# NVIDIA-Merlin/models

Hardware: NVIDIA H100
Metric: DLRM fwd samples/sec (Criteo shape, batch 65536/GPU) (higher is better)
Workload: dtype fp32 I/O; GEMM-shaped work as split-bf16 x3 (hi*hi + hi*lo + lo*hi, fp32 accumulate, |err| ~ 2^-16)

## Files before the change

### models_b200/csrc/mlp_tc.cu

```cuda
#include <cuda.h>
#include <cuda_bf16.h>

#include <cstring>

#include "mm_common.cuh"
#include "tc_common.cuh"

namespace mm {
namespace mlp {

using namespace mm::tc;

constexpr int BLOCK_M = 128;
constexpr int BLOCK_K = 64;
constexpr int MMA_K = 16;
constexpr int kConsumerWarps = 8;
constexpr int kThreads = 32 * (kConsumerWarps + 1);
constexpr int kMaxChain = 3;
constexpr int kMaxHeads = 8;
constexpr uint32_t A_TILE_BYTES = BLOCK_M * BLOCK_K * 2;

struct ChainLayer {
  int N, Np;
  int Kp;
  int act;
  uint32_t w_off;
};

struct Params {
  long long M;
  int K1p, N1, N1p, act1, stages, n_chain;
  ChainLayer c[kMaxChain];
  const float* bias[kMaxChain + 1];
  uint32_t w_bytes;
  float* out_f32;
  uint8_t* out_operand;
  long long out_stride;
  const float* head_w;
  float head_b;
  int head_act;
  float* head_out;
  int n_heads;
  const float* heads_w;
  const float* heads_b;
  int heads_act[kMaxHeads];
  float* heads_out;
};

template <int NP, int KS>
__device__ __forceinline__ void chain_mma(float (&acc)[64], const uint32_t (&ahi)[32], const uint32_t (&alo)[32], uint32_t w_hi,
                                          uint32_t w_lo, uint32_t tile_b) {
  wgmma_fence();
#pragma unroll
  for (int ks = 0; ks < KS; ++ks) {
    const uint32_t f[4] = {ahi[4 * ks], ahi[4 * ks + 1], ahi[4 * ks + 2], ahi[4 * ks + 3]};
    wgmma_rs(NP, acc, f, make_desc_sw128(w_lo + (ks >> 2) * tile_b + (ks & 3) * 32));
  }
#pragma unroll
  for (int ks = 0; ks < KS; ++ks) {
    const uint32_t f[4] = {alo[4 * ks], alo[4 * ks + 1], alo[4 * ks + 2], alo[4 * ks + 3]};
    wgmma_rs(NP, acc, f, make_desc_sw128(w_hi + (ks >> 2) * tile_b + (ks & 3) * 32));
  }
#pragma unroll
  for (int ks = 0; ks < KS; ++ks) {
    const uint32_t f[4] = {ahi[4 * ks], ahi[4 * ks + 1], ahi[4 * ks + 2], ahi[4 * ks + 3]};
    wgmma_rs(NP, acc, f, make_desc_sw128(w_hi + (ks >> 2) * tile_b + (ks & 3) * 32));
  }
  wgmma_commit();
  wgmma_wait_all();
}
template <int KS>
__device__ __forceinline__ void chain_mma(int np, float (&acc)[64], const uint32_t (&ahi)[32], const uint32_t (&alo)[32],
                                          uint32_t w_hi, uint32_t w_lo, uint32_t tile_b) {
  switch (np) {
    case 16: chain_mma<16, KS>(acc, ahi, alo, w_hi, w_lo, tile_b); break;
    case 32: chain_mma<32, KS>(acc, ahi, alo, w_hi, w_lo, tile_b); break;
    case 48: chain_mma<48, KS>(acc, ahi, alo, w_hi, w_lo, tile_b); break;
    case 64: chain_mma<64, KS>(acc, ahi, alo, w_hi, w_lo, tile_b); break;
    case 80: chain_mma<80, KS>(acc, ahi, alo, w_hi, w_lo, tile_b); break;
    case 96: chain_mma<96, KS>(acc, ahi, alo, w_hi, w_lo, tile_b); break;
    case 112: chain_mma<112, KS>(acc, ahi, alo, w_hi, w_lo, tile_b); break;
    default: chain_mma<128, KS>(acc, ahi, alo, w_hi, w_lo, tile_b); break;
  }
}

template <int N1P, bool HEADS>
__global__ void __launch_bounds__(kThreads, 1)
mlp_tc_kernel(const __grid_constant__ CUtensorMap tmA, const __grid_constant__ CUtensorMap tmW1,
              const __grid_constant__ CUtensorMap tmC0, const __grid_constant__ CUtensorMap tmC1,
              const __grid_constant__ CUtensorMap tmC2, const Params p) {
  extern __shared__ __align__(1024) uint8_t smem_raw[];
  uint8_t* smem = smem_raw + ((1024u - (smem_u32(smem_raw) & 1023u)) & 1023u);
  constexpr uint32_t B_TILE_BYTES = (uint32_t)N1P * BLOCK_K * 2;
  constexpr uint32_t STAGE_BYTES = A_TILE_BYTES + B_TILE_BYTES;
  uint8_t* wres = smem + (size_t)p.stages * STAGE_BYTES;
  uint64_t* bars = reinterpret_cast<uint64_t*>(wres + p.w_bytes);
  uint64_t* full_bar = bars;
  uint64_t* empty_bar = bars + p.stages;
  uint64_t* w_full = bars + 2 * p.stages;
  float* bias_s = reinterpret_cast<float*>(bars + 2 * p.stages + 2);
  float* head_s = bias_s + (kMaxChain + 1) * 128;

  const int warp = threadIdx.x >> 5, lane = threadIdx.x & 31;
  const long long tiles = (p.M + BLOCK_M - 1) / BLOCK_M;
  const int KB = p.K1p / BLOCK_K;

  if (warp == kConsumerWarps && lane == 0) {
    asm volatile("prefetch.tensormap [%0];" ::"l"(&tmA) : "memory");
    asm volatile("prefetch.tensormap [%0];" ::"l"(&tmW1) : "memory");
    for (int s = 0; s < p.stages; ++s) {
      mbar_init(smem_u32(full_bar + s), 1);
      mbar_init(smem_u32(empty_bar + s), kConsumerWarps);
    }
    mbar_init(smem_u32(w_full), 1);
    asm volatile("fence.mbarrier_init.release.cluster;" ::: "memory");
  }
  for (int i = threadIdx.x; i < (kMaxChain + 1) * 128; i += kThreads) {
    const int l = i >> 7, n = i & 127;
    const int N = l == 0 ? p.N1 : (l <= p.n_chain ? p.c[l - 1].N : 0);
    bias_s[i] = (p.bias[l] != nullptr && n < N) ? p.bias[l][n] : 0.0f;
  }
  if (HEADS) {
    const int Nl = p.n_chain ? p.c[p.n_chain - 1].N : p.N1;
    for (int i = threadIdx.x; i < kMaxHeads * 128; i += kThreads) {
      const int hh = i >> 7, n = i & 127;
      head_s[i] = (hh < p.n_heads && n < Nl) ? p.heads_w[n * p.n_heads + hh] : 0.0f;
    }
    if (threadIdx.x < kMaxHeads)
      head_s[kMaxHeads * 128 + threadIdx.x] = ((int)threadIdx.x < p.n_heads && p.heads_b) ? p.heads_b[threadIdx.x] : 0.0f;
  } else if (threadIdx.x < 128) {
    const int Nl = p.n_chain ? p.c[p.n_chain - 1].N : p.N1;
    head_s[threadIdx.x] = (p.head_w != nullptr && (int)threadIdx.x < Nl) ? p.head_w[threadIdx.x] : 0.0f;
  }
  __syncthreads();

  if (warp == kConsumerWarps) {
    if (lane == 0) {
      if (p.n_chain > 0) {
        const uint32_t wb = smem_u32(w_full);
        mbar_expect_tx(wb, p.w_bytes);
        for (int c = 0; c < p.n_chain; ++c) {
          const CUtensorMap* tm = c == 0 ? &tmC0 : (c == 1 ? &tmC1 : &tmC2);
          const uint32_t tile_b = (uint32_t)p.c[c].Np * BLOCK_K * 2;
          const int kbs = p.c[c].Kp / BLOCK_K;
          for (int kb = 0; kb < kbs; ++kb) {
            tma_load_2d(smem_u32(wres + p.c[c].w_off + (size_t)kb * tile_b), tm, wb, kb * BLOCK_K, 0);
            tma_load_2d(smem_u32(wres + p.c[c].w_off + (size_t)(kbs + kb) * tile_b), tm, wb, p.c[c].Kp + kb * BLOCK_K, 0);
          }
        }
      }
      int stage = 0;
      uint32_t phase = 0;
      for (long long tile = blockIdx.x; tile < tiles; tile += gridDim.x) {
        const int m0 = (int)tile * BLOCK_M;
        for (int kb2 = 0; kb2 < 2 * KB; ++kb2) {
          const int kb = kb2 >> 1, col = (kb2 & 1) * p.K1p + kb * BLOCK_K;
          mbar_wait(smem_u32(empty_bar + stage), phase ^ 1);
          const uint32_t fb = smem_u32(full_bar + stage);
          uint8_t* st = smem + (size_t)stage * STAGE_BYTES;
          mbar_expect_tx(fb, STAGE_BYTES);
          tma_load_2d(smem_u32(st), &tmA, fb, col, m0);
          tma_load_2d(smem_u32(st + A_TILE_BYTES), &tmW1, fb, col, 0);
          if (++stage == p.stages) {
            stage = 0;
            phase ^= 1;
          }
        }
      }
    }
  } else {
    const int wg = warp >> 2;
    const int c2 = 2 * (lane & 3);
    const int frow = 64 * wg + 16 * (warp & 3) + (lane >> 2);
    const uint32_t a_off = (uint32_t)wg * (A_TILE_BYTES / 2);
    int stage = 0;
    uint32_t phase = 0;
    bool weights_ready = p.n_chain == 0;
    for (long long tile = blockIdx.x; tile < tiles; tile += gridDim.x) {
      float acc[64];
#pragma unroll
      for (int i = 0; i < 64; ++i) acc[i] = 0.0f;
      for (int kb = 0; kb < KB; ++kb) {
        const int s_hi = stage;
        mbar_wait(smem_u32(full_bar + s_hi), phase);
        const uint32_t a_hi = smem_u32(smem + (size_t)s_hi * STAGE_BYTES), b_hi = a_hi + A_TILE_BYTES;
        wgmma_fence_acc(acc);
        wgmma_fence();
#pragma unroll
        for (int k = 0; k < BLOCK_K / MMA_K; ++k)
          wgmma_ss(N1P, acc, make_desc_sw128(a_hi + a_off + k * 32), make_desc_sw128(b_hi + k * 32));
        wgmma_commit();
        if (++stage == p.stages) {
          stage = 0;
          phase ^= 1;
        }
        const int s_lo = stage;
        mbar_wait(smem_u32(full_bar + s_lo), phase);
        const uint32_t a_lo = smem_u32(smem + (size_t)s_lo * STAGE_BYTES), b_lo = a_lo + A_TILE_BYTES;
        wgmma_fence();
#pragma unroll
        for (int k = 0; k < BLOCK_K / MMA_K; ++k)
          wgmma_ss(N1P, acc, make_desc_sw128(a_hi + a_off + k * 32), make_desc_sw128(b_lo + k * 32));
#pragma unroll
        for (int k = 0; k < BLOCK_K / MMA_K; ++k)
          wgmma_ss(N1P, acc, make_desc_sw128(a_lo + a_off + k * 32), make_desc_sw128(b_hi + k * 32));
        wgmma_commit();
        wgmma_wait_all();
        wgmma_fence_acc(acc);
        __syncwarp();
        if (lane == 0) {
          mbar_arrive(smem_u32(empty_bar + s_hi));
          mbar_arrive(smem_u32(empty_bar + s_lo));
        }
        if (++stage == p.stages) {
          stage = 0;
          phase ^= 1;
        }
      }

      for (int layer = 0; layer <= p.n_chain; ++layer) {
        const bool last = layer == p.n_chain;
        const int N = layer == 0 ? p.N1 : p.c[layer - 1].N;
        const int Np = layer == 0 ? N1P : p.c[layer - 1].Np;
        const int act = layer == 0 ? p.act1 : p.c[layer - 1].act;
        const float* bs = bias_s + layer * 128;
#pragma unroll
        for (int j = 0; j < 16; ++j) {
          if (8 * j < Np) {
#pragma unroll
            for (int e = 0; e < 4; ++e) {
              const int col = 8 * j + c2 + (e & 1);
              float v = acc[4 * j + e] + bs[col];
              if (act == MM_ACT_RELU) v = fmaxf(v, 0.0f);
              else if (act != MM_ACT_LINEAR && col < N) v = apply_act_slow(v, act);
              acc[4 * j + e] = col < N ? v : 0.0f;
            }
          }
        }
        if (!last) {
          uint32_t ahi[32], alo[32];
#pragma unroll
          for (int i = 0; i < 32; ++i) split_pair(acc[2 * i], acc[2 * i + 1], ahi[i], alo[i]);
          const ChainLayer& L = p.c[layer];
          if (!weights_ready) {
            mbar_wait(smem_u32(w_full), 0);
            weights_ready = true;
          }
          const uint32_t tile_b = (uint32_t)L.Np * BLOCK_K * 2;
          const uint32_t w_hi = smem_u32(wres + L.w_off), w_lo = w_hi + (uint32_t)(L.Kp / BLOCK_K) * tile_b;
#pragma unroll
          for (int i = 0; i < 64; ++i) acc[i] = 0.0f;
          wgmma_fence_acc(acc);
          if (L.Kp == BLOCK_K) chain_mma<BLOCK_K / MMA_K>(L.Np, acc, ahi, alo, w_hi, w_lo, tile_b);
          else chain_mma<2 * BLOCK_K / MMA_K>(L.Np, acc, ahi, alo, w_hi, w_lo, tile_b);
          wgmma_fence_acc(acc);
        } else {
#pragma unroll
          for (int h = 0; h < 2; ++h) {
            const long long row = tile * BLOCK_M + frow + 8 * h;
            if (HEADS) {
#pragma unroll
              for (int hh = 0; hh < kMaxHeads; ++hh) {
                if (hh < p.n_heads) {
                  const float* hw = head_s + hh * 128;
                  float hsum = 0.0f;
#pragma unroll
                  for (int j = 0; j < 4; ++j) {
                    hsum = fmaf(acc[4 * j + 2 * h], hw[8 * j + c2], hsum);
                    hsum = fmaf(acc[4 * j + 2 * h + 1], hw[8 * j + c2 + 1], hsum);
                  }
                  hsum += __shfl_xor_sync(0xffffffffu, hsum, 1);
                  hsum += __shfl_xor_sync(0xffffffffu, hsum, 2);
                  if ((lane & 3) == 0 && row < p.M)
                    p.heads_out[hh * p.M + row] = apply_act(hsum + head_s[kMaxHeads * 128 + hh], p.heads_act[hh]);
                }
              }
            } else if (p.head_w) {
              float hsum = 0.0f;
#pragma unroll
              for (int j = 0; j < 4; ++j) {
                hsum = fmaf(acc[4 * j + 2 * h], head_s[8 * j + c2], hsum);
                hsum = fmaf(acc[4 * j + 2 * h + 1], head_s[8 * j + c2 + 1], hsum);
              }
              hsum += __shfl_xor_sync(0xffffffffu, hsum, 1);
              hsum += __shfl_xor_sync(0xffffffffu, hsum, 2);
              if ((lane & 3) == 0 && row < p.M) p.head_out[row] = apply_act(hsum + p.head_b, p.head_act);
            }
            if (row < p.M && (p.out_f32 || p.out_operand)) {
#pragma unroll
              for (int j = 0; j < 16; ++j) {
                const int n = 8 * j + c2;
                if (8 * j < Np && n < N) {
                  const float x = acc[4 * j + 2 * h], y = acc[4 * j + 2 * h + 1];
                  if (p.out_operand) {
                    uint32_t hi, lo;
                    split_pair(x, y, hi, lo);
                    uint8_t* rowp = p.out_operand + row * ((long long)N * 4);
                    *reinterpret_cast<uint32_t*>(rowp + n * 2) = hi;
                    *reinterpret_cast<uint32_t*>(rowp + N * 2 + n * 2) = lo;
                  }
                  if (p.out_f32) {
                    float* g = p.out_f32 + row * p.out_stride + n;
                    g[0] = x;
                    if (n + 1 < N) g[1] = y;
                  }
                }
              }
            }
          }
        }
      }
    }
  }
}

}
}

static bool plan_tower(int K, int n_layers, const int* widths, mm::mlp::Params& p, size_t& smem, bool heads = false) {
  using namespace mm::mlp;
  memset(&p, 0, sizeof(p));
  p.K1p = mm_tc_padded_k(K);
  p.N1 = widths[0];
  p.N1p = mm_tc_padded_n(widths[0]);
  p.n_chain = n_layers - 1;
  uint32_t w_off = 0;
  int prev_n = p.N1;
  for (int c = 0; c < p.n_chain; ++c) {
    ChainLayer& L = p.c[c];
    L.N = widths[c + 1];
    L.Np = mm_tc_padded_n(L.N);
    L.Kp = mm_tc_padded_k(prev_n);
    L.w_off = w_off;
    w_off += (uint32_t)(2 * (L.Kp / BLOCK_K)) * (uint32_t)L.Np * BLOCK_K * 2;
    prev_n = L.N;
  }
  p.w_bytes = w_off;
  const size_t stage_bytes = (size_t)A_TILE_BYTES + (size_t)p.N1p * BLOCK_K * 2;
  const size_t head_floats = heads ? kMaxHeads * 128 + kMaxHeads : 128;
  const size_t fixed = 1024 + (size_t)p.w_bytes + 40 * sizeof(uint64_t) + ((kMaxChain + 1) * 128 + head_floats) * sizeof(float);
  if (fixed + 4 * stage_bytes > 227 * 1024) return false;
  int stages = (int)((227 * 1024 - fixed) / stage_bytes);
  if (stages > 12) stages = 12;
  const int kb1 = p.K1p / BLOCK_K;
  if (stages > 4 * kb1) stages = 4 * kb1 > 4 ? 4 * kb1 : 4;
  p.stages = stages;
  smem = 1024 + stages * stage_bytes + p.w_bytes + (2 * stages + 2) * sizeof(uint64_t) +
         ((kMaxChain + 1) * 128 + head_floats) * sizeof(float);
  return true;
}

extern "C" {

int mm_mlp_tc_supported(int K, int n_layers, const int* widths, int with_head) {
  if (K <= 0 || !widths || n_layers < 2 || n_layers > mm::mlp::kMaxChain + 1) return 0;
  for (int l = 0; l < n_layers; ++l)
    if (widths[l] < 1 || widths[l] > 128) return 0;
  if (with_head && widths[n_layers - 1] > 32) return 0;
  mm::mlp::Params p;
  size_t smem = 0;
  return plan_tower(K, n_layers, widths, p, smem, with_head > 1) ? 1 : 0;
}

}

typedef void (*MlpKernel)(const CUtensorMap, const CUtensorMap, const CUtensorMap, const CUtensorMap, const CUtensorMap,
                          const mm::mlp::Params);

template <bool HEADS>
static MlpKernel kernel_for(int n1p) {
  using namespace mm::mlp;
  switch (n1p) {
    case 16: return mlp_tc_kernel<16, HEADS>;
    case 32: return mlp_tc_kernel<32, HEADS>;
    case 48: return mlp_tc_kernel<48, HEADS>;
    case 64: return mlp_tc_kernel<64, HEADS>;
    case 80: return mlp_tc_kernel<80, HEADS>;
    case 96: return mlp_tc_kernel<96, HEADS>;
    case 112: return mlp_tc_kernel<112, HEADS>;
    case 128: return mlp_tc_kernel<128, HEADS>;
  }
  return nullptr;
}

static int mlp_tc_impl(const void* a_split, int64_t M, int K, int n_layers, const void* const* w_split, const int* widths,
                       const float* const* bias, const int* acts, float* out, int64_t out_stride, const float* head_w,
                       float head_b, int head_act, float* head_out, void* out_operand, void* stream,
                       int n_heads = 0, const float* heads_b = nullptr, const int* heads_act = nullptr) {
  using namespace mm::mlp;
  MM_REQUIRE(a_split && w_split && widths && bias && acts && M >= 0 && K > 0, MM_ERR_ARG, "mm_mlp_tc: null pointer or bad M/K");
  MM_REQUIRE(n_layers >= 1 && n_layers <= kMaxChain + 1, MM_ERR_UNSUPPORTED, "mm_mlp_tc: 1..%d layers (got %d)", kMaxChain + 1,
             n_layers);
  MM_REQUIRE(out || head_out || out_operand, MM_ERR_ARG, "mm_mlp_tc: no output requested");
  MM_REQUIRE(!out_operand || (widths[n_layers - 1] % 4 == 0 && ((uintptr_t)out_operand % 16) == 0 &&
                              (!out || ((out_stride & 3) == 0 && ((uintptr_t)out % 16) == 0))),
             MM_ERR_ALIGN, "mm_mlp_tc: operand-format output needs a last width that is a multiple of 4 and 16-B aligned outputs");
  MM_REQUIRE((head_w == nullptr) == (head_out == nullptr), MM_ERR_ARG, "mm_mlp_tc: head weights and head output go together");
  MM_REQUIRE(((uintptr_t)a_split % 16) == 0, MM_ERR_ALIGN, "mm_mlp_tc: a_split must be 16-B aligned");
  MM_REQUIRE(M < (1ll << 31), MM_ERR_UNSUPPORTED, "mm_mlp_tc: M too large for 32-bit TMA coordinates");
  for (int l = 0; l < n_layers; ++l) {
    MM_REQUIRE(w_split[l] && ((uintptr_t)w_split[l] % 16) == 0, MM_ERR_ARG, "mm_mlp_tc: layer %d weights null or misaligned", l);
    MM_REQUIRE(widths[l] >= 1 && widths[l] <= 128, MM_ERR_UNSUPPORTED, "mm_mlp_tc: layer %d width %d is not in 1..128", l,
               widths[l]);
    MM_REQUIRE(acts[l] >= MM_ACT_LINEAR && acts[l] <= MM_ACT_GELU, MM_ERR_ARG, "mm_mlp_tc: unknown activation %d", acts[l]);
  }
  const int n_last = widths[n_layers - 1];
  MM_REQUIRE(!head_w || n_last <= 32, MM_ERR_UNSUPPORTED, "mm_mlp_tc: the fused Dense(N->1) head needs a last width <= 32");
  MM_REQUIRE(!head_w || n_heads || (head_act >= MM_ACT_LINEAR && head_act <= MM_ACT_GELU), MM_ERR_ARG,
             "mm_mlp_tc: unknown head activation");
  for (int hh = 0; hh < n_heads; ++hh)
    MM_REQUIRE(heads_act[hh] >= MM_ACT_LINEAR && heads_act[hh] <= MM_ACT_GELU, MM_ERR_ARG, "mm_mlp_tc_heads: unknown activation of head %d",
               hh);
  MM_REQUIRE(!out || out_stride >= n_last, MM_ERR_ARG, "mm_mlp_tc: out_stride < last width");
  if (M == 0) return MM_OK;

  Params p;
  size_t smem = 0;
  MM_REQUIRE(plan_tower(K, n_layers, widths, p, smem, n_heads > 0), MM_ERR_UNSUPPORTED,
             "mm_mlp_tc: the tower does not fit in shared memory with two pipeline stages (mm_mlp_tc_supported)");
  p.M = M;
  p.act1 = acts[0];
  for (int l = 0; l < n_layers; ++l) p.bias[l] = bias[l];
  for (int c = 0; c < p.n_chain; ++c) p.c[c].act = acts[c + 1];
  p.out_f32 = out;
  p.out_stride = out_stride;
  p.out_operand = (uint8_t*)out_operand;
  p.head_w = head_w;
  p.head_b = head_b;
  p.head_act = head_act;
  p.head_out = head_out;
  if (n_heads > 0) {
    p.head_w = nullptr;
    p.head_out = nullptr;
    p.n_heads = n_heads;
    p.heads_w = head_w;
    p.heads_b = heads_b;
    for (int hh = 0; hh < n_heads; ++hh) p.heads_act[hh] = heads_act[hh];
    p.heads_out = head_out;
  }

  CUtensorMap tmA, tmW1, tmC[kMaxChain];
  int rc = mm::tc::make_map(&tmA, a_split, (uint64_t)M, (uint64_t)2 * p.K1p, BLOCK_M);
  if (rc) return rc;
  rc = mm::tc::make_map(&tmW1, w_split[0], (uint64_t)p.N1p, (uint64_t)2 * p.K1p, (uint32_t)p.N1p);
  if (rc) return rc;
  for (int c = 0; c < kMaxChain; ++c) {
    if (c < p.n_chain) {
      rc = mm::tc::make_map(&tmC[c], w_split[c + 1], (uint64_t)p.c[c].Np, (uint64_t)2 * p.c[c].Kp, (uint32_t)p.c[c].Np);
      if (rc) return rc;
    } else {
      tmC[c] = tmW1;
    }
  }

  MlpKernel kern = n_heads > 0 ? kernel_for<true>(p.N1p) : kernel_for<false>(p.N1p);
  MM_REQUIRE(kern != nullptr, MM_ERR_UNSUPPORTED, "mm_mlp_tc: no kernel for a padded layer-1 width of %d", p.N1p);
  static bool smem_set[2][8] = {};
  if (!smem_set[n_heads > 0][p.N1p / 16 - 1]) {
    cudaError_t e = cudaFuncSetAttribute(kern, cudaFuncAttributeMaxDynamicSharedMemorySize, 227 * 1024);
    if (e != cudaSuccess) {
      mm::set_error("mm_mlp_tc: cudaFuncSetAttribute(227 KB smem) failed: %s", cudaGetErrorString(e));
      return (int)e;
    }
    smem_set[n_heads > 0][p.N1p / 16 - 1] = true;
  }
  const long long tiles = (M + BLOCK_M - 1) / BLOCK_M;
  const int sms = mm::sm_count();
  const unsigned grid = (unsigned)(tiles < sms ? tiles : sms);
  kern<<<grid, kThreads, smem, (cudaStream_t)stream>>>(tmA, tmW1, tmC[0], tmC[1], tmC[2], p);
  return mm::check_launch("mm_mlp_tc");
}

extern "C" {

int mm_mlp_tc(const void* a_split, int64_t M, int K, int n_layers, const void* const* w_split, const int* widths,
              const float* const* bias, const int* acts, float* out, int64_t out_stride, const float* head_w,
              float head_b, int head_act, float* head_out, void* stream) {
  return mlp_tc_impl(a_split, M, K, n_layers, w_split, widths, bias, acts, out, out_stride, head_w, head_b, head_act, head_out,
                     nullptr, stream);
}

int mm_mlp_tc_heads(const void* a_split, int64_t M, int K, int n_layers, const void* const* w_split, const int* widths,
                    const float* const* bias, const int* acts, int n_heads, const float* heads_w, const float* heads_b,
                    const int* heads_act, float* heads_out, void* stream) {
  MM_REQUIRE(n_heads >= 1 && n_heads <= mm::mlp::kMaxHeads, MM_ERR_UNSUPPORTED, "mm_mlp_tc_heads: %d heads is not in 1..%d", n_heads,
             mm::mlp::kMaxHeads);
  MM_REQUIRE(heads_w && heads_out && heads_act, MM_ERR_ARG, "mm_mlp_tc_heads: null heads_w / heads_act / heads_out");
  return mlp_tc_impl(a_split, M, K, n_layers, w_split, widths, bias, acts, nullptr, 0, heads_w, 0.0f, 0, heads_out, nullptr, stream,
                     n_heads, heads_b, heads_act);
}

int mm_mlp_tc_operand_out(const void* a_split, int64_t M, int K, int n_layers, const void* const* w_split, const int* widths,
                          const float* const* bias, const int* acts, float* out, int64_t out_stride, void* out_operand,
                          void* stream) {
  MM_REQUIRE(out_operand != nullptr, MM_ERR_ARG, "mm_mlp_tc_operand_out: out_operand is null");
  return mlp_tc_impl(a_split, M, K, n_layers, w_split, widths, bias, acts, out, out_stride, nullptr, 0.0f, 0, nullptr, out_operand,
                     stream);
}

}
```

### models_b200/csrc/tc_common.cuh

```cuda
#pragma once
#include <cuda.h>
#include <cuda_bf16.h>

#include "mm_common.cuh"
#include "warp_mma.cuh"

namespace mm {
namespace tc {

__device__ __forceinline__ void mbar_init(uint32_t bar, uint32_t count) {
  asm volatile("mbarrier.init.shared::cta.b64 [%0], %1;" ::"r"(bar), "r"(count) : "memory");
}
__device__ __forceinline__ void mbar_expect_tx(uint32_t bar, uint32_t bytes) {
  asm volatile("mbarrier.arrive.expect_tx.shared::cta.b64 _, [%0], %1;" ::"r"(bar), "r"(bytes) : "memory");
}
__device__ __forceinline__ void mbar_arrive(uint32_t bar) {
  asm volatile("mbarrier.arrive.shared::cta.b64 _, [%0];" ::"r"(bar) : "memory");
}
__device__ __forceinline__ void mbar_wait(uint32_t bar, uint32_t parity) {
  uint32_t ok = 0, spins = 0;
  const long long t0 = clock64();
  while (true) {
    asm volatile(
        "{\n .reg .pred p;\n mbarrier.try_wait.parity.shared::cta.b64 p, [%1], %2;\n selp.u32 %0, 1, 0, p;\n}"
        : "=r"(ok)
        : "r"(bar), "r"(parity)
        : "memory");
    if (ok) return;
    if ((++spins & 1023u) == 0u && clock64() - t0 > 8000000000ll) __trap();
  }
}
__device__ __forceinline__ void tma_load_2d(uint32_t dst, const CUtensorMap* map, uint32_t bar, int c0, int c1) {
  asm volatile(
      "cp.async.bulk.tensor.2d.shared::cta.global.mbarrier::complete_tx::bytes [%0], [%1, {%3, %4}], [%2];" ::"r"(dst),
      "l"(map), "r"(bar), "r"(c0), "r"(c1)
      : "memory");
}
__device__ __forceinline__ void wgmma_fence() { asm volatile("wgmma.fence.sync.aligned;" ::: "memory"); }
__device__ __forceinline__ void wgmma_commit() { asm volatile("wgmma.commit_group.sync.aligned;" ::: "memory"); }
__device__ __forceinline__ void wgmma_wait_all() { asm volatile("wgmma.wait_group.sync.aligned 0;" ::: "memory"); }
__device__ __forceinline__ void wgmma_fence_acc(float (&d)[64]) {
#pragma unroll
  for (int i = 0; i < 64; ++i) asm volatile("" : "+f"(d[i])::"memory");
}
__device__ __forceinline__ void named_bar(int id, int threads) {
  asm volatile("bar.sync %0, %1;" ::"r"(id), "r"(threads) : "memory");
}

__device__ __forceinline__ void wgmma_ss_n16(float (&d)[64], uint64_t a, uint64_t b) {
  asm volatile(
      "{\n wgmma.mma_async.sync.aligned.m64n16k16.f32.bf16.bf16 "
      "{%0, %1, %2, %3, %4, %5, %6, %7}, %8, %9, 1, 1, 1, 0, 0;\n}"
      : "+f"(d[0]), "+f"(d[1]), "+f"(d[2]), "+f"(d[3]), "+f"(d[4]), "+f"(d[5]), "+f"(d[6]), "+f"(d[7])
      : "l"(a), "l"(b));
}
__device__ __forceinline__ void wgmma_rs_n16(float (&d)[64], const uint32_t (&a)[4], uint64_t b) {
  asm volatile(
      "{\n wgmma.mma_async.sync.aligned.m64n16k16.f32.bf16.bf16 "
      "{%0, %1, %2, %3, %4, %5, %6, %7}, {%8, %9, %10, %11}, %12, 1, 1, 1, 0;\n}"
      : "+f"(d[0]), "+f"(d[1]), "+f"(d[2]), "+f"(d[3]), "+f"(d[4]), "+f"(d[5]), "+f"(d[6]), "+f"(d[7])
      : "r"(a[0]), "r"(a[1]), "r"(a[2]), "r"(a[3]), "l"(b));
}
__device__ __forceinline__ void wgmma_ss_n32(float (&d)[64], uint64_t a, uint64_t b) {
  asm volatile(
      "{\n wgmma.mma_async.sync.aligned.m64n32k16.f32.bf16.bf16 "
      "{%0, %1, %2, %3, %4, %5, %6, %7, %8, %9, %10, %11, %12, %13, %14, %15}, %16, %17, 1, 1, 1, 0, 0;\n}"
      : "+f"(d[0]), "+f"(d[1]), "+f"(d[2]), "+f"(d[3]), "+f"(d[4]), "+f"(d[5]), "+f"(d[6]), "+f"(d[7]), "+f"(d[8]), "+f"(d[9]), "+f"(d[10]), "+f"(d[11]), "+f"(d[12]), "+f"(d[13]), "+f"(d[14]), "+f"(d[15])
      : "l"(a), "l"(b));
}
__device__ __forceinline__ void wgmma_rs_n32(float (&d)[64], const uint32_t (&a)[4], uint64_t b) {
  asm volatile(
      "{\n wgmma.mma_async.sync.aligned.m64n32k16.f32.bf16.bf16 "
      "{%0, %1, %2, %3, %4, %5, %6, %7, %8, %9, %10, %11, %12, %13, %14, %15}, {%16, %17, %18, %19}, %20, 1, 1, 1, 0;\n}"
      : "+f"(d[0]), "+f"(d[1]), "+f"(d[2]), "+f"(d[3]), "+f"(d[4]), "+f"(d[5]), "+f"(d[6]), "+f"(d[7]), "+f"(d[8]), "+f"(d[9]), "+f"(d[10]), "+f"(d[11]), "+f"(d[12]), "+f"(d[13]), "+f"(d[14]), "+f"(d[15])
      : "r"(a[0]), "r"(a[1]), "r"(a[2]), "r"(a[3]), "l"(b));
}
__device__ __forceinline__ void wgmma_ss_n48(float (&d)[64], uint64_t a, uint64_t b) {
  asm volatile(
      "{\n wgmma.mma_async.sync.aligned.m64n48k16.f32.bf16.bf16 "
      "{%0, %1, %2, %3, %4, %5, %6, %7, %8, %9, %10, %11, %12, %13, %14, %15, %16, %17, %18, %19, %20, %21, %22, %23}, %24, %25, 1, 1, 1, 0, 0;\n}"
      : "+f"(d[0]), "+f"(d[1]), "+f"(d[2]), "+f"(d[3]), "+f"(d[4]), "+f"(d[5]), "+f"(d[6]), "+f"(d[7]), "+f"(d[8]), "+f"(d[9]), "+f"(d[10]), "+f"(d[11]), "+f"(d[12]), "+f"(d[13]), "+f"(d[14]), "+f"(d[15]), "+f"(d[16]), "+f"(d[17]), "+f"(d[18]), "+f"(d[19]), "+f"(d[20]), "+f"(d[21]), "+f"(d[22]), "+f"(d[23])
      : "l"(a), "l"(b));
}
__device__ __forceinline__ void wgmma_rs_n48(float (&d)[64], const uint32_t (&a)[4], uint64_t b) {
  asm volatile(
      "{\n wgmma.mma_async.sync.aligned.m64n48k16.f32.bf16.bf16 "
      "{%0, %1, %2, %3, %4, %5, %6, %7, %8, %9, %10, %11, %12, %13, %14, %15, %16, %17, %18, %19, %20, %21, %22, %23}, {%24, %25, %26, %27}, %28, 1, 1, 1, 0;\n}"
      : "+f"(d[0]), "+f"(d[1]), "+f"(d[2]), "+f"(d[3]), "+f"(d[4]), "+f"(d[5]), "+f"(d[6]), "+f"(d[7]), "+f"(d[8]), "+f"(d[9]), "+f"(d[10]), "+f"(d[11]), "+f"(d[12]), "+f"(d[13]), "+f"(d[14]), "+f"(d[15]), "+f"(d[16]), "+f"(d[17]), "+f"(d[18]), "+f"(d[19]), "+f"(d[20]), "+f"(d[21]), "+f"(d[22]), "+f"(d[23])
      : "r"(a[0]), "r"(a[1]), "r"(a[2]), "r"(a[3]), "l"(b));
}
__device__ __forceinline__ void wgmma_ss_n64(float (&d)[64], uint64_t a, uint64_t b) {
  asm volatile(
      "{\n wgmma.mma_async.sync.aligned.m64n64k16.f32.bf16.bf16 "
      "{%0, %1, %2, %3, %4, %5, %6, %7, %8, %9, %10, %11, %12, %13, %14, %15, %16, %17, %18, %19, %20, %21, %22, %23, %24, %25, %26, %27, %28, %29, %30, %31}, %32, %33, 1, 1, 1, 0, 0;\n}"
      : "+f"(d[0]), "+f"(d[1]), "+f"(d[2]), "+f"(d[3]), "+f"(d[4]), "+f"(d[5]), "+f"(d[6]), "+f"(d[7]), "+f"(d[8]), "+f"(d[9]), "+f"(d[10]), "+f"(d[11]), "+f"(d[12]), "+f"(d[13]), "+f"(d[14]), "+f"(d[15]), "+f"(d[16]), "+f"(d[17]), "+f"(d[18]), "+f"(d[19]), "+f"(d[20]), "+f"(d[21]), "+f"(d[22]), "+f"(d[23]), "+f"(d[24]), "+f"(d[25]), "+f"(d[26]), "+f"(d[27]), "+f"(d[28]), "+f"(d[29]), "+f"(d[30]), "+f"(d[31])
      : "l"(a), "l"(b));
}
__device__ __forceinline__ void wgmma_rs_n64(float (&d)[64], const uint32_t (&a)[4], uint64_t b) {
  asm volatile(
      "{\n wgmma.mma_async.sync.aligned.m64n64k16.f32.bf16.bf16 "
      "{%0, %1, %2, %3, %4, %5, %6, %7, %8, %9, %10, %11, %12, %13, %14, %15, %16, %17, %18, %19, %20, %21, %22, %23, %24, %25, %26, %27, %28, %29, %30, %31}, {%32, %33, %34, %35}, %36, 1, 1, 1, 0;\n}"
      : "+f"(d[0]), "+f"(d[1]), "+f"(d[2]), "+f"(d[3]), "+f"(d[4]), "+f"(d[5]), "+f"(d[6]), "+f"(d[7]), "+f"(d[8]), "+f"(d[9]), "+f"(d[10]), "+f"(d[11]), "+f"(d[12]), "+f"(d[13]), "+f"(d[14]), "+f"(d[15]), "+f"(d[16]), "+f"(d[17]), "+f"(d[18]), "+f"(d[19]), "+f"(d[20]), "+f"(d[21]), "+f"(d[22]), "+f"(d[23]), "+f"(d[24]), "+f"(d[25]), "+f"(d[26]), "+f"(d[27]), "+f"(d[28]), "+f"(d[29]), "+f"(d[30]), "+f"(d[31])
      : "r"(a[0]), "r"(a[1]), "r"(a[2]), "r"(a[3]), "l"(b));
}
__device__ __forceinline__ void wgmma_ss_n80(float (&d)[64], uint64_t a, uint64_t b) {
  asm volatile(
      "{\n wgmma.mma_async.sync.aligned.m64n80k16.f32.bf16.bf16 "
      "{%0, %1, %2, %3, %4, %5, %6, %7, %8, %9, %10, %11, %12, %13, %14, %15, %16, %17, %18, %19, %20, %21, %22, %23, %24, %25, %26, %27, %28, %29, %30, %31, %32, %33, %34, %35, %36, %37, %38, %39}, %40, %41, 1, 1, 1, 0, 0;\n}"
      : "+f"(d[0]), "+f"(d[1]), "+f"(d[2]), "+f"(d[3]), "+f"(d[4]), "+f"(d[5]), "+f"(d[6]), "+f"(d[7]), "+f"(d[8]), "+f"(d[9]), "+f"(d[10]), "+f"(d[11]), "+f"(d[12]), "+f"(d[13]), "+f"(d[14]), "+f"(d[15]), "+f"(d[16]), "+f"(d[17]), "+f"(d[18]), "+f"(d[19]), "+f"(d[20]), "+f"(d[21]), "+f"(d[22]), "+f"(d[23]), "+f"(d[24]), "+f"(d[25]), "+f"(d[26]), "+f"(d[27]), "+f"(d[28]), "+f"(d[29]), "+f"(d[30]), "+f"(d[31]), "+f"(d[32]), "+f"(d[33]), "+f"(d[34]), "+f"(d[35]), "+f"(d[36]), "+f"(d[37]), "+f"(d[38]), "+f"(d[39])
      : "l"(a), "l"(b));
}
__device__ __forceinline__ void wgmma_rs_n80(float (&d)[64], const uint32_t (&a)[4], uint64_t b) {
  asm volatile(
      "{\n wgmma.mma_async.sync.aligned.m64n80k16.f32.bf16.bf16 "
      "{%0, %1, %2, %3, %4, %5, %6, %7, %8, %9, %10, %11, %12, %13, %14, %15, %16, %17, %18, %19, %20, %21, %22, %23, %24, %25, %26, %27, %28, %29, %30, %31, %32, %33, %34, %35, %36, %37, %38, %39}, {%40, %41, %42, %43}, %44, 1, 1, 1, 0;\n}"
      : "+f"(d[0]), "+f"(d[1]), "+f"(d[2]), "+f"(d[3]), "+f"(d[4]), "+f"(d[5]), "+f"(d[6]), "+f"(d[7]), "+f"(d[8]), "+f"(d[9]), "+f"(d[10]), "+f"(d[11]), "+f"(d[12]), "+f"(d[13]), "+f"(d[14]), "+f"(d[15]), "+f"(d[16]), "+f"(d[17]), "+f"(d[18]), "+f"(d[19]), "+f"(d[20]), "+f"(d[21]), "+f"(d[22]), "+f"(d[23]), "+f"(d[24]), "+f"(d[25]), "+f"(d[26]), "+f"(d[27]), "+f"(d[28]), "+f"(d[29]), "+f"(d[30]), "+f"(d[31]), "+f"(d[32]), "+f"(d[33]), "+f"(d[34]), "+f"(d[35]), "+f"(d[36]), "+f"(d[37]), "+f"(d[38]), "+f"(d[39])
      : "r"(a[0]), "r"(a[1]), "r"(a[2]), "r"(a[3]), "l"(b));
}
__device__ __forceinline__ void wgmma_ss_n96(float (&d)[64], uint64_t a, uint64_t b) {
  asm volatile(
      "{\n wgmma.mma_async.sync.aligned.m64n96k16.f32.bf16.bf16 "
      "{%0, %1, %2, %3, %4, %5, %6, %7, %8, %9, %10, %11, %12, %13, %14, %15, %16, %17, %18, %19, %20, %21, %22, %23, %24, %25, %26, %27, %28, %29, %30, %31, %32, %33, %34, %35, %36, %37, %38, %39, %40, %41, %42, %43, %44, %45, %46, %47}, %48, %49, 1, 1, 1, 0, 0;\n}"
      : "+f"(d[0]), "+f"(d[1]), "+f"(d[2]), "+f"(d[3]), "+f"(d[4]), "+f"(d[5]), "+f"(d[6]), "+f"(d[7]), "+f"(d[8]), "+f"(d[9]), "+f"(d[10]), "+f"(d[11]), "+f"(d[12]), "+f"(d[13]), "+f"(d[14]), "+f"(d[15]), "+f"(d[16]), "+f"(d[17]), "+f"(d[18]), "+f"(d[19]), "+f"(d[20]), "+f"(d[21]), "+f"(d[22]), "+f"(d[23]), "+f"(d[24]), "+f"(d[25]), "+f"(d[26]), "+f"(d[27]), "+f"(d[28]), "+f"(d[29]), "+f"(d[30]), "+f"(d[31]), "+f"(d[32]), "+f"(d[33]), "+f"(d[34]), "+f"(d[35]), "+f"(d[36]), "+f"(d[37]), "+f"(d[38]), "+f"(d[39]), "+f"(d[40]), "+f"(d[41]), "+f"(d[42]), "+f"(d[43]), "+f"(d[44]), "+f"(d[45]), "+f"(d[46]), "+f"(d[47])
      : "l"(a), "l"(b));
}
__device__ __forceinline__ void wgmma_rs_n96(float (&d)[64], const uint32_t (&a)[4], uint64_t b) {
  asm volatile(
      "{\n wgmma.mma_async.sync.aligned.m64n96k16.f32.bf16.bf16 "
      "{%0, %1, %2, %3, %4, %5, %6, %7, %8, %9, %10, %11, %12, %13, %14, %15, %16, %17, %18, %19, %20, %21, %22, %23, %24, %25, %26, %27, %28, %29, %30, %31, %32, %33, %34, %35, %36, %37, %38, %39, %40, %41, %42, %43, %44, %45, %46, %47}, {%48, %49, %50, %51}, %52, 1, 1, 1, 0;\n}"
      : "+f"(d[0]), "+f"(d[1]), "+f"(d[2]), "+f"(d[3]), "+f"(d[4]), "+f"(d[5]), "+f"(d[6]), "+f"(d[7]), "+f"(d[8]), "+f"(d[9]), "+f"(d[10]), "+f"(d[11]), "+f"(d[12]), "+f"(d[13]), "+f"(d[14]), "+f"(d[15]), "+f"(d[16]), "+f"(d[17]), "+f"(d[18]), "+f"(d[19]), "+f"(d[20]), "+f"(d[21]), "+f"(d[22]), "+f"(d[23]), "+f"(d[24]), "+f"(d[25]), "+f"(d[26]), "+f"(d[27]), "+f"(d[28]), "+f"(d[29]), "+f"(d[30]), "+f"(d[31]), "+f"(d[32]), "+f"(d[33]), "+f"(d[34]), "+f"(d[35]), "+f"(d[36]), "+f"(d[37]), "+f"(d[38]), "+f"(d[39]), "+f"(d[40]), "+f"(d[41]), "+f"(d[42]), "+f"(d[43]), "+f"(d[44]), "+f"(d[45]), "+f"(d[46]), "+f"(d[47])
      : "r"(a[0]), "r"(a[1]), "r"(a[2]), "r"(a[3]), "l"(b));
}
__device__ __forceinline__ void wgmma_ss_n112(float (&d)[64], uint64_t a, uint64_t b) {
  asm volatile(
      "{\n wgmma.mma_async.sync.aligned.m64n112k16.f32.bf16.bf16 "
      "{%0, %1, %2, %3, %4, %5, %6, %7, %8, %9, %10, %11, %12, %13, %14, %15, %16, %17, %18, %19, %20, %21, %22, %23, %24, %25, %26, %27, %28, %29, %30, %31, %32, %33, %34, %35, %36, %37, %38, %39, %40, %41, %42, %43, %44, %45, %46, %47, %48, %49, %50, %51, %52, %53, %54, %55}, %56, %57, 1, 1, 1, 0, 0;\n}"
      : "+f"(d[0]), "+f"(d[1]), "+f"(d[2]), "+f"(d[3]), "+f"(d[4]), "+f"(d[5]), "+f"(d[6]), "+f"(d[7]), "+f"(d[8]), "+f"(d[9]), "+f"(d[10]), "+f"(d[11]), "+f"(d[12]), "+f"(d[13]), "+f"(d[14]), "+f"(d[15]), "+f"(d[16]), "+f"(d[17]), "+f"(d[18]), "+f"(d[19]), "+f"(d[20]), "+f"(d[21]), "+f"(d[22]), "+f"(d[23]), "+f"(d[24]), "+f"(d[25]), "+f"(d[26]), "+f"(d[27]), "+f"(d[28]), "+f"(d[29]), "+f"(d[30]), "+f"(d[31]), "+f"(d[32]), "+f"(d[33]), "+f"(d[34]), "+f"(d[35]), "+f"(d[36]), "+f"(d[37]), "+f"(d[38]), "+f"(d[39]), "+f"(d[40]), "+f"(d[41]), "+f"(d[42]), "+f"(d[43]), "+f"(d[44]), "+f"(d[45]), "+f"(d[46]), "+f"(d[47]), "+f"(d[48]), "+f"(d[49]), "+f"(d[50]), "+f"(d[51]), "+f"(d[52]), "+f"(d[53]), "+f"(d[54]), "+f"(d[55])
      : "l"(a), "l"(b));
}
__device__ __forceinline__ void wgmma_rs_n112(float (&d)[64], const uint32_t (&a)[4], uint64_t b) {
  asm volatile(
      "{\n wgmma.mma_async.sync.aligned.m64n112k16.f32.bf16.bf16 "
      "{%0, %1, %2, %3, %4, %5, %6, %7, %8, %9, %10, %11, %12, %13, %14, %15, %16, %17, %18, %19, %20, %21, %22, %23, %24, %25, %26, %27, %28, %29, %30, %31, %32, %33, %34, %35, %36, %37, %38, %39, %40, %41, %42, %43, %44, %45, %46, %47, %48, %49, %50, %51, %52, %53, %54, %55}, {%56, %57, %58, %59}, %60, 1, 1, 1, 0;\n}"
      : "+f"(d[0]), "+f"(d[1]), "+f"(d[2]), "+f"(d[3]), "+f"(d[4]), "+f"(d[5]), "+f"(d[6]), "+f"(d[7]), "+f"(d[8]), "+f"(d[9]), "+f"(d[10]), "+f"(d[11]), "+f"(d[12]), "+f"(d[13]), "+f"(d[14]), "+f"(d[15]), "+f"(d[16]), "+f"(d[17]), "+f"(d[18]), "+f"(d[19]), "+f"(d[20]), "+f"(d[21]), "+f"(d[22]), "+f"(d[23]), "+f"(d[24]), "+f"(d[25]), "+f"(d[26]), "+f"(d[27]), "+f"(d[28]), "+f"(d[29]), "+f"(d[30]), "+f"(d[31]), "+f"(d[32]), "+f"(d[33]), "+f"(d[34]), "+f"(d[35]), "+f"(d[36]), "+f"(d[37]), "+f"(d[38]), "+f"(d[39]), "+f"(d[40]), "+f"(d[41]), "+f"(d[42]), "+f"(d[43]), "+f"(d[44]), "+f"(d[45]), "+f"(d[46]), "+f"(d[47]), "+f"(d[48]), "+f"(d[49]), "+f"(d[50]), "+f"(d[51]), "+f"(d[52]), "+f"(d[53]), "+f"(d[54]), "+f"(d[55])
      : "r"(a[0]), "r"(a[1]), "r"(a[2]), "r"(a[3]), "l"(b));
}
__device__ __forceinline__ void wgmma_ss_n128(float (&d)[64], uint64_t a, uint64_t b) {
  asm volatile(
      "{\n wgmma.mma_async.sync.aligned.m64n128k16.f32.bf16.bf16 "
      "{%0, %1, %2, %3, %4, %5, %6, %7, %8, %9, %10, %11, %12, %13, %14, %15, %16, %17, %18, %19, %20, %21, %22, %23, %24, %25, %26, %27, %28, %29, %30, %31, %32, %33, %34, %35, %36, %37, %38, %39, %40, %41, %42, %43, %44, %45, %46, %47, %48, %49, %50, %51, %52, %53, %54, %55, %56, %57, %58, %59, %60, %61, %62, %63}, %64, %65, 1, 1, 1, 0, 0;\n}"
      : "+f"(d[0]), "+f"(d[1]), "+f"(d[2]), "+f"(d[3]), "+f"(d[4]), "+f"(d[5]), "+f"(d[6]), "+f"(d[7]), "+f"(d[8]), "+f"(d[9]), "+f"(d[10]), "+f"(d[11]), "+f"(d[12]), "+f"(d[13]), "+f"(d[14]), "+f"(d[15]), "+f"(d[16]), "+f"(d[17]), "+f"(d[18]), "+f"(d[19]), "+f"(d[20]), "+f"(d[21]), "+f"(d[22]), "+f"(d[23]), "+f"(d[24]), "+f"(d[25]), "+f"(d[26]), "+f"(d[27]), "+f"(d[28]), "+f"(d[29]), "+f"(d[30]), "+f"(d[31]), "+f"(d[32]), "+f"(d[33]), "+f"(d[34]), "+f"(d[35]), "+f"(d[36]), "+f"(d[37]), "+f"(d[38]), "+f"(d[39]), "+f"(d[40]), "+f"(d[41]), "+f"(d[42]), "+f"(d[43]), "+f"(d[44]), "+f"(d[45]), "+f"(d[46]), "+f"(d[47]), "+f"(d[48]), "+f"(d[49]), "+f"(d[50]), "+f"(d[51]), "+f"(d[52]), "+f"(d[53]), "+f"(d[54]), "+f"(d[55]), "+f"(d[56]), "+f"(d[57]), "+f"(d[58]), "+f"(d[59]), "+f"(d[60]), "+f"(d[61]), "+f"(d[62]), "+f"(d[63])
      : "l"(a), "l"(b));
}
__device__ __forceinline__ void wgmma_rs_n128(float (&d)[64], const uint32_t (&a)[4], uint64_t b) {
  asm volatile(
      "{\n wgmma.mma_async.sync.aligned.m64n128k16.f32.bf16.bf16 "
      "{%0, %1, %2, %3, %4, %5, %6, %7, %8, %9, %10, %11, %12, %13, %14, %15, %16, %17, %18, %19, %20, %21, %22, %23, %24, %25, %26, %27, %28, %29, %30, %31, %32, %33, %34, %35, %36, %37, %38, %39, %40, %41, %42, %43, %44, %45, %46, %47, %48, %49, %50, %51, %52, %53, %54, %55, %56, %57, %58, %59, %60, %61, %62, %63}, {%64, %65, %66, %67}, %68, 1, 1, 1, 0;\n}"
      : "+f"(d[0]), "+f"(d[1]), "+f"(d[2]), "+f"(d[3]), "+f"(d[4]), "+f"(d[5]), "+f"(d[6]), "+f"(d[7]), "+f"(d[8]), "+f"(d[9]), "+f"(d[10]), "+f"(d[11]), "+f"(d[12]), "+f"(d[13]), "+f"(d[14]), "+f"(d[15]), "+f"(d[16]), "+f"(d[17]), "+f"(d[18]), "+f"(d[19]), "+f"(d[20]), "+f"(d[21]), "+f"(d[22]), "+f"(d[23]), "+f"(d[24]), "+f"(d[25]), "+f"(d[26]), "+f"(d[27]), "+f"(d[28]), "+f"(d[29]), "+f"(d[30]), "+f"(d[31]), "+f"(d[32]), "+f"(d[33]), "+f"(d[34]), "+f"(d[35]), "+f"(d[36]), "+f"(d[37]), "+f"(d[38]), "+f"(d[39]), "+f"(d[40]), "+f"(d[41]), "+f"(d[42]), "+f"(d[43]), "+f"(d[44]), "+f"(d[45]), "+f"(d[46]), "+f"(d[47]), "+f"(d[48]), "+f"(d[49]), "+f"(d[50]), "+f"(d[51]), "+f"(d[52]), "+f"(d[53]), "+f"(d[54]), "+f"(d[55]), "+f"(d[56]), "+f"(d[57]), "+f"(d[58]), "+f"(d[59]), "+f"(d[60]), "+f"(d[61]), "+f"(d[62]), "+f"(d[63])
      : "r"(a[0]), "r"(a[1]), "r"(a[2]), "r"(a[3]), "l"(b));
}
__device__ __forceinline__ void wgmma_ss(int n, float (&d)[64], uint64_t a, uint64_t b) {
  switch (n) {
    case 16: wgmma_ss_n16(d, a, b); break;
    case 32: wgmma_ss_n32(d, a, b); break;
    case 48: wgmma_ss_n48(d, a, b); break;
    case 64: wgmma_ss_n64(d, a, b); break;
    case 80: wgmma_ss_n80(d, a, b); break;
    case 96: wgmma_ss_n96(d, a, b); break;
    case 112: wgmma_ss_n112(d, a, b); break;
    case 128: wgmma_ss_n128(d, a, b); break;
  }
}
__device__ __forceinline__ void wgmma_rs(int n, float (&d)[64], const uint32_t (&a)[4], uint64_t b) {
  switch (n) {
    case 16: wgmma_rs_n16(d, a, b); break;
    case 32: wgmma_rs_n32(d, a, b); break;
    case 48: wgmma_rs_n48(d, a, b); break;
    case 64: wgmma_rs_n64(d, a, b); break;
    case 80: wgmma_rs_n80(d, a, b); break;
    case 96: wgmma_rs_n96(d, a, b); break;
    case 112: wgmma_rs_n112(d, a, b); break;
    case 128: wgmma_rs_n128(d, a, b); break;
  }
}

__device__ __forceinline__ uint64_t make_desc_sw128(uint32_t smem_addr) {
  uint64_t d = 0;
  d |= (uint64_t)((smem_addr & 0x3FFFF) >> 4);
  d |= (uint64_t)1 << 16;
  d |= (uint64_t)(1024 >> 4) << 32;
  d |= (uint64_t)1 << 62;
  return d;
}

typedef CUresult (*EncodeTiledFn)(CUtensorMap*, CUtensorMapDataType, cuuint32_t, void*, const cuuint64_t*,
                                  const cuuint64_t*, const cuuint32_t*, const cuuint32_t*, CUtensorMapInterleave,
                                  CUtensorMapSwizzle, CUtensorMapL2promotion, CUtensorMapFloatOOBfill);

static inline EncodeTiledFn encode_fn() {
  static EncodeTiledFn fn = nullptr;
  static bool tried = false;
  if (!tried) {
    tried = true;
    void* p = nullptr;
    cudaDriverEntryPointQueryResult q;
    if (cudaGetDriverEntryPoint("cuTensorMapEncodeTiled", &p, cudaEnableDefault, &q) == cudaSuccess &&
        q == cudaDriverEntryPointSuccess)
      fn = reinterpret_cast<EncodeTiledFn>(p);
  }
  return fn;
}

static inline int make_map(CUtensorMap* map, const void* base, uint64_t rows, uint64_t cols, uint32_t box_rows) {
  EncodeTiledFn fn = encode_fn();
  MM_REQUIRE(fn != nullptr, MM_ERR_DRIVER, "cuTensorMapEncodeTiled is not available from the driver");
  cuuint64_t dims[2] = {cols, rows};
  cuuint64_t strides[1] = {cols * 2};
  cuuint32_t box[2] = {64u, box_rows};
  cuuint32_t estr[2] = {1, 1};
  CUresult r = fn(map, CU_TENSOR_MAP_DATA_TYPE_BFLOAT16, 2, const_cast<void*>(base), dims, strides, box, estr,
                  CU_TENSOR_MAP_INTERLEAVE_NONE, CU_TENSOR_MAP_SWIZZLE_128B, CU_TENSOR_MAP_L2_PROMOTION_L2_256B,
                  CU_TENSOR_MAP_FLOAT_OOB_FILL_NONE);
  MM_REQUIRE(r == CUDA_SUCCESS, MM_ERR_DRIVER, "cuTensorMapEncodeTiled failed with CUresult %d", (int)r);
  return MM_OK;
}

}
}
```

Measured before the change: 294.4 million.

## Split consumer warpgroups onto alternating 64-row tiles with ping-pong named barriers

Halves BLOCK_M to 64 so each consumer warpgroup processes its own tile, with the two warpgroups taking alternate tiles. Named barriers hand the smem pipeline back and forth so one group's epilogue and chained layers overlap the other's first-layer GEMM. Each group works out its stage and phase from the tile index. It also adds a specialised ReLU epilogue that reads the bias as float2 and drops the Np branch. Risks include smaller wgmma tiles, more TMA requests per row, named-barrier deadlock if tile counts are uneven, and an out-of-range bias read if Np is below 128.

```diff
diff --git a/models_b200/csrc/mlp_tc.cu b/models_b200/csrc/mlp_tc.cu
--- a/models_b200/csrc/mlp_tc.cu
+++ b/models_b200/csrc/mlp_tc.cu
@@ -11,13 +11,14 @@
 
 using namespace mm::tc;
 
-constexpr int BLOCK_M = 128;
+constexpr int BLOCK_M = 64;
 constexpr int BLOCK_K = 64;
 constexpr int MMA_K = 16;
 constexpr int kConsumerWarps = 8;
 constexpr int kThreads = 32 * (kConsumerWarps + 1);
 constexpr int kMaxChain = 3;
 constexpr int kMaxHeads = 8;
+constexpr int kTurnBar = 1;
 constexpr uint32_t A_TILE_BYTES = BLOCK_M * BLOCK_K * 2;
 
 struct ChainLayer {
@@ -110,7 +111,7 @@
     asm volatile("prefetch.tensormap [%0];" ::"l"(&tmW1) : "memory");
     for (int s = 0; s < p.stages; ++s) {
       mbar_init(smem_u32(full_bar + s), 1);
-      mbar_init(smem_u32(empty_bar + s), kConsumerWarps);
+      mbar_init(smem_u32(empty_bar + s), kConsumerWarps / 2);
     }
     mbar_init(smem_u32(w_full), 1);
     asm volatile("fence.mbarrier_init.release.cluster;" ::: "memory");
@@ -171,15 +172,16 @@
   } else {
     const int wg = warp >> 2;
     const int c2 = 2 * (lane & 3);
-    const int frow = 64 * wg + 16 * (warp & 3) + (lane >> 2);
-    const uint32_t a_off = (uint32_t)wg * (A_TILE_BYTES / 2);
-    int stage = 0;
-    uint32_t phase = 0;
+    const int frow = 16 * (warp & 3) + (lane >> 2);
     bool weights_ready = p.n_chain == 0;
-    for (long long tile = blockIdx.x; tile < tiles; tile += gridDim.x) {
+    for (long long tile = blockIdx.x + (long long)wg * gridDim.x; tile < tiles; tile += 2ll * gridDim.x) {
+      const long long pos = (tile - blockIdx.x) / gridDim.x * (2 * KB);
+      int stage = (int)(pos % p.stages);
+      uint32_t phase = (uint32_t)(pos / p.stages) & 1u;
       float acc[64];
 #pragma unroll
       for (int i = 0; i < 64; ++i) acc[i] = 0.0f;
+      if (tile >= (long long)blockIdx.x + gridDim.x) named_bar(kTurnBar + wg, 256);
       for (int kb = 0; kb < KB; ++kb) {
         const int s_hi = stage;
         mbar_wait(smem_u32(full_bar + s_hi), phase);
@@ -188,7 +190,7 @@
         wgmma_fence();
 #pragma unroll
         for (int k = 0; k < BLOCK_K / MMA_K; ++k)
-          wgmma_ss(N1P, acc, make_desc_sw128(a_hi + a_off + k * 32), make_desc_sw128(b_hi + k * 32));
+          wgmma_ss(N1P, acc, make_desc_sw128(a_hi + k * 32), make_desc_sw128(b_hi + k * 32));
         wgmma_commit();
         if (++stage == p.stages) {
           stage = 0;
@@ -200,10 +202,10 @@
         wgmma_fence();
 #pragma unroll
         for (int k = 0; k < BLOCK_K / MMA_K; ++k)
-          wgmma_ss(N1P, acc, make_desc_sw128(a_hi + a_off + k * 32), make_desc_sw128(b_lo + k * 32));
+          wgmma_ss(N1P, acc, make_desc_sw128(a_hi + k * 32), make_desc_sw128(b_lo + k * 32));
 #pragma unroll
         for (int k = 0; k < BLOCK_K / MMA_K; ++k)
-          wgmma_ss(N1P, acc, make_desc_sw128(a_lo + a_off + k * 32), make_desc_sw128(b_hi + k * 32));
+          wgmma_ss(N1P, acc, make_desc_sw128(a_lo + k * 32), make_desc_sw128(b_hi + k * 32));
         wgmma_commit();
         wgmma_wait_all();
         wgmma_fence_acc(acc);
@@ -217,6 +219,7 @@
           phase ^= 1;
         }
       }
+      if (tile + gridDim.x < tiles) named_bar_arrive(kTurnBar + (wg ^ 1), 256);
 
       for (int layer = 0; layer <= p.n_chain; ++layer) {
         const bool last = layer == p.n_chain;
@@ -224,15 +227,25 @@
         const int Np = layer == 0 ? N1P : p.c[layer - 1].Np;
         const int act = layer == 0 ? p.act1 : p.c[layer - 1].act;
         const float* bs = bias_s + layer * 128;
-#pragma unroll
-        for (int j = 0; j < 16; ++j) {
-          if (8 * j < Np) {
+        if (act == MM_ACT_RELU) {
+#pragma unroll
+          for (int j = 0; j < 16; ++j) {
+            const float2 b = *reinterpret_cast<const float2*>(bs + 8 * j + c2);
+#pragma unroll
+            for (int e = 0; e < 4; ++e) {
+              const int col = 8 * j + c2 + (e & 1);
+              const float v = fmaxf(acc[4 * j + e] + ((e & 1) ? b.y : b.x), 0.0f);
+              acc[4 * j + e] = col < N ? v : 0.0f;
+            }
+          }
+        } else {
+#pragma unroll
+          for (int j = 0; j < 16; ++j) {
 #pragma unroll
             for (int e = 0; e < 4; ++e) {
               const int col = 8 * j + c2 + (e & 1);
               float v = acc[4 * j + e] + bs[col];
-              if (act == MM_ACT_RELU) v = fmaxf(v, 0.0f);
-              else if (act != MM_ACT_LINEAR && col < N) v = apply_act_slow(v, act);
+              if (act != MM_ACT_LINEAR && col < N) v = apply_act_slow(v, act);
               acc[4 * j + e] = col < N ? v : 0.0f;
             }
           }
diff --git a/models_b200/csrc/tc_common.cuh b/models_b200/csrc/tc_common.cuh
--- a/models_b200/csrc/tc_common.cuh
+++ b/models_b200/csrc/tc_common.cuh
@@ -45,6 +45,9 @@
 }
 __device__ __forceinline__ void named_bar(int id, int threads) {
   asm volatile("bar.sync %0, %1;" ::"r"(id), "r"(threads) : "memory");
+}
+__device__ __forceinline__ void named_bar_arrive(int id, int threads) {
+  asm volatile("bar.arrive %0, %1;" ::"r"(id), "r"(threads) : "memory");
 }
 
 __device__ __forceinline__ void wgmma_ss_n16(float (&d)[64], uint64_t a, uint64_t b) {
```

After: 311.2 million (median of 6 runs). 1.06x the previous value.
